# rosielab/emojivoice

Measured on AMD Instinct MI355X. Metric: audio_seconds_per_second, higher is better.
Workload: dtype f32 (deep layers: operand = two block-scaled fp16 pieces, product = 3 fp16 products on the fp16 MFMA, f32 accumulate); 1 GPU; config2: batch 64 x 516-frame (5.99 s) utterances per GPU, 10 Euler steps + HiFi-GAN V1, 22.05 kHz; global_batch=64, frames=516, ode_steps=10, parallelism=dp1, collective=none, batch_pipeline=cfm(i+1) || hifigan(i) on two streams, 2 pipeline(s) in flight

## Files before the change

emojivoice_amd/_lib.py:

```python
from __future__ import annotations

import ctypes as C
import math
import os
import subprocess
from typing import Dict, Optional

import numpy as np
import torch

_HERE = os.path.dirname(os.path.abspath(__file__))
LIB_PATH = os.environ.get("EV_LIB_PATH") or os.path.join(_HERE, "lib", "libemojivoice_hip.so")
CSRC = os.path.join(_HERE, "csrc")
SOURCES = [os.path.join(CSRC, n) for n in ("ev_engine.hip", "ev_kernels.h", "ev_analysis_kernels.h", "ev_analysis.h")] \
    + [os.path.join(os.path.dirname(_HERE), "include", "emojivoice.h")]

EXPORTS = [
    "ev_abi_version", "ev_create", "ev_destroy", "ev_last_error", "ev_load_estimator", "ev_load_vocoder", "ev_load_vocoder_cfg", "ev_load_text_encoder", "ev_text_encoder",
    "ev_text_encoder_status", "ev_stft_magnitude", "ev_denoise", "ev_align", "ev_dbg_conv_bench",
    "ev_workspace_bytes", "ev_cfm_decode", "ev_estimator", "ev_hifigan", "ev_profile_enable", "ev_profile_read", "ev_profile_read_split", "ev_dbg_last_cfg", "ev_set_arithmetic", "ev_get_arithmetic",
    "ev_op_conv1d", "ev_op_groupnorm_mish", "ev_op_groupnorm_mish2", "ev_op_conv_groupnorm", "ev_op_layernorm", "ev_op_split_pieces", "ev_op_attention", "ev_op_ln_mlp", "ev_set_mrf_streams_max",
    "ev_cfm_decode2", "ev_reserve", "ev_alloc_count", "ev_dbg_sk_stats", "ev_op_attn_out", "ev_dbg_set_amax", "ev_dbg_set_attn_h16", "ev_dbg_set_chain", "ev_dbg_sk_taken",
    "ev_load_mel_basis", "ev_mel_spectrogram",
    "ev_maximum_path", "ev_log_prior", "ev_mas_align",
    "ev_estimator_rows", "ev_cfm_loss",
    "ev_load_resampler", "ev_resample", "ev_mel_stats",
    "ev_trim_bounds", "ev_trim_apply",
    "ev_pitch_yin", "ev_dtw",
    "ev_loudness",
    "ev_pyin_observe", "ev_pyin_decode",
    "ev_op_attention2", "ev_op_attn_out2",
    "ev_load_stoi", "ev_stoi",
    "ev_load_stft_dist", "ev_stft_dist",
    "ev_load_voice_quality", "ev_voice_quality",
    "ev_load_formants", "ev_formants", "ev_formant_track",
    "ev_perturbation",
    "ev_load_harmonics", "ev_harmonics",
    "ev_functionals",
    "ev_load_auditory", "ev_auditory",
]


class EvLibraryError(RuntimeError):
    pass

# ... 114 lines not shown
    lib.ev_load_voice_quality.argtypes = [vp, vp, vp, i32, i32, i32, vp, vp, i32, i32, i32, vp, C.c_double]
    lib.ev_voice_quality.argtypes = [vp, vp, vp, i32, i32, C.c_double, vp, vp, vp, vp]
    lib.ev_load_formants.argtypes = [vp, vp, i32, i32, i32, C.c_double, C.c_double, C.c_double, i32]
    lib.ev_formants.argtypes = [vp, vp, vp, i32, i32, C.c_double, vp, vp, vp, vp]
    lib.ev_formant_track.argtypes = [vp, vp, vp, i32, i32, i32, i32, vp, C.c_double, C.c_double, C.c_double, vp, vp, vp, vp, vp]
    lib.ev_perturbation.argtypes = [vp, vp, vp, i32, i32, i32, vp, i32, i32, C.c_double, C.c_double, C.c_double, vp, vp, vp, vp]
    lib.ev_load_harmonics.argtypes = [vp, vp, vp, i32, i32, i32, C.c_double, i32, C.c_double, C.c_double, C.c_double]
    lib.ev_harmonics.argtypes = [vp, vp, vp, i32, i32, vp, vp, vp, i32, C.c_double, vp, vp, vp, vp]
    lib.ev_functionals.argtypes = [vp, vp, vp, vp, i32, i32, i32, vp, i32, vp, vp, vp]
    lib.ev_load_auditory.argtypes = [vp, vp, vp, i32, i32, i32, vp, i32, vp, vp, i32, i32, i32, C.c_double]
    lib.ev_auditory.argtypes = [vp, vp, vp, i32, i32, C.c_double, vp, vp, vp, vp, vp]
    lib.ev_maximum_path.argtypes = [vp, vp, vp, vp, i32, i32, i32, vp, vp, vp]
    lib.ev_log_prior.argtypes = [vp, vp, vp, i32, i32, i32, vp, vp]
    lib.ev_mas_align.argtypes = [vp, vp, vp, vp, vp, i32, i32, i32, vp, vp, vp, vp, vp]
    lib.ev_profile_enable.argtypes = [vp, i32]
    lib.ev_profile_read.argtypes = [vp, C.POINTER(C.c_double), C.POINTER(C.c_double), C.POINTER(C.c_int64), i32]
    lib.ev_profile_read_split.argtypes = [vp, C.POINTER(C.c_double), C.POINTER(C.c_double), C.POINTER(C.c_int64)]
    lib.ev_dbg_last_cfg.argtypes = [vp]
    lib.ev_set_arithmetic.argtypes = [vp, i32]
    lib.ev_get_arithmetic.argtypes = [vp]
    lib.ev_dbg_set_amax.argtypes = [vp, i32]
    lib.ev_dbg_set_attn_h16.argtypes = [vp, i32]
    lib.ev_dbg_set_chain.argtypes = [vp, i32]
    lib.ev_dbg_sk_taken.argtypes = [vp]
    lib.ev_dbg_sk_taken.restype = C.c_int64
    lib.ev_op_conv1d.argtypes = [vp, vp, vp, vp, i32, i32, i32, i32, i32, i32, i32, i32, i32, f32, vp, vp]
    lib.ev_op_groupnorm_mish.argtypes = [vp, vp, vp, vp, vp, i32, i32, i32, i32, vp, vp]
    lib.ev_op_groupnorm_mish2.argtypes = [vp, vp, vp, vp, vp, i32, i32, i32, i32, i32, vp, i32, vp, vp, vp]
    lib.ev_op_conv_groupnorm.argtypes = [vp, vp, vp, vp, i32, i32, i32, vp, vp, vp, i32, vp, vp, vp, vp, vp, C.POINTER(C.c_int), vp]
    lib.ev_op_layernorm.argtypes = [vp, vp, vp, vp, i32, i32, vp, vp]
    lib.ev_op_split_pieces.argtypes = [vp, vp, i32, vp, vp]
    lib.ev_op_attention.argtypes = [vp, vp, vp, i32, i32, i32, vp, vp]
    lib.ev_op_attn_out.argtypes = [vp, vp, vp, i32, i32, vp, vp, vp, vp]
    lib.ev_op_attention2.argtypes = [vp, vp, vp, i32, i32, i32, i32, i32, i32, vp, C.POINTER(C.c_int), vp]
    lib.ev_op_attn_out2.argtypes = [vp, vp, vp, i32, i32, i32, i32, vp, vp, f32, f32, f32, vp, C.POINTER(C.c_int), vp]
    lib.ev_op_ln_mlp.argtypes = [vp, vp, vp, vp, vp, vp, vp, vp, vp, vp, vp, i32, i32, i32, vp, vp]
    for n in EXPORTS:
        getattr(lib, n)
    _lib = lib
    return lib


def _stream_ptr() -> int:
    return int(torch.cuda.current_stream().cuda_stream)


# ... 671 lines not shown
        for b0 in range(0, B, bmax):
            b1 = min(B, b0 + bmax)
            self._check(self.lib.ev_hifigan(self.h, mel[b0:b1].data_ptr(), b1 - b0, T, wav[b0:b1].data_ptr(), _stream_ptr()), "ev_hifigan")
        return wav

    def workspace_bytes(self, B: int, Tp: int, Tv: int) -> int:
        return int(self.lib.ev_workspace_bytes(self.h, B, Tp, Tv))

    def profile_enable(self, on: bool):
        self._check(self.lib.ev_profile_enable(self.h, int(on)), "ev_profile_enable")

    def op_split_pieces(self, x):
        x = self._f32(x).reshape(-1)
        out = torch.empty((3, x.numel()), dtype=torch.float32, device=x.device)
        self._check(self.lib.ev_op_split_pieces(self.h, x.data_ptr(), x.numel(), out.data_ptr(), _stream_ptr()), "ev_op_split_pieces")
        return out

    def set_arithmetic(self, bf16_products: int):
        self._check(self.lib.ev_set_arithmetic(self.h, int(bf16_products)), "ev_set_arithmetic")

    def set_amax(self, on: bool) -> None:
        self._check(self.lib.ev_dbg_set_amax(self.h, int(bool(on))), "ev_dbg_set_amax")

    def set_attn_h16(self, on: bool) -> None:
        self._check(self.lib.ev_dbg_set_attn_h16(self.h, int(bool(on))), "ev_dbg_set_attn_h16")

    def set_chain(self, on: bool) -> None:
        self._check(self.lib.ev_dbg_set_chain(self.h, int(bool(on))), "ev_dbg_set_chain")

    def arithmetic(self) -> int:
        return int(self.lib.ev_get_arithmetic(self.h))

    def last_cfg(self) -> int:
        return int(self.lib.ev_dbg_last_cfg(self.h))

    def profile_read_split(self):
        ms, fl, n = C.c_double(), C.c_double(), C.c_int64()
        self._check(self.lib.ev_profile_read_split(self.h, C.byref(ms), C.byref(fl), C.byref(n)), "ev_profile_read_split")
        return ms.value, fl.value, n.value

    def profile_read(self, reset: bool = True):
        ms, fl, n = C.c_double(), C.c_double(), C.c_int64()
        self._check(self.lib.ev_profile_read(self.h, C.byref(ms), C.byref(fl), C.byref(n), int(reset)), "ev_profile_read")
        return ms.value, fl.value, n.value

    def op_conv1d(self, x, w, bias, dilation=1, transposed=False, stride=1, padding=0, pre_lrelu_slope=-1.0):
# ... 145 lines not shown
```

emojivoice_amd/csrc/ev_engine.hip:

```cpp
#include "ev_kernels.h"
#include "../../include/emojivoice.h"

#include <math.h>
#include <stdlib.h>
#include <stdarg.h>
#include <stdio.h>
#include <string.h>

#include <algorithm>
#include <atomic>
#include <mutex>
#include <numeric>
#include <string>
#include <unordered_map>
#include <vector>

namespace {

struct HostTensor {
    const float* p = nullptr;
    int ndim = 0;
    int64_t shape[4] = {0, 0, 0, 0};
    int64_t numel() const { int64_t n = 1; for (int i = 0; i < ndim; ++i) n *= shape[i]; return n; }
};
// ... 10 lines not shown
    int2* taplist[3] = {nullptr, nullptr, nullptr};
    int* nact[3] = {nullptr, nullptr, nullptr};
    bool sparse_taps = false;
    bool tile128_exact = true;
    int kstack_mt = 0, kstack_tap = 0;
    int ntaps = 0, off[EV_MAX_TAPS] = {0};
    int halo_lo = 0, halo_hi = 0;
    bool wide = false;
    int Cin = 0, Cout = 0, Mpad = 0, Kpad = 0;
    double macs_per_row = 0;
};

struct Epi {
    int act = ACT_NONE; float act_slope = 0.f; const float* act_a = nullptr; const float* act_b = nullptr;
    int mask1 = 0; float scale = 1.f; const float* R = nullptr; int ldr = 0; int accum = 0; int div3 = 0;
    int act2_lrelu = 0; float act2_slope = 0.f; int mask2 = 0; const float* rowmask = nullptr; int mmul = 1;
    float* Y2 = nullptr; int ldy2 = 0;
    float pro_slope = -1.f;
    int dbg = 0; int force_cfg = -1; int stagger = -1; unsigned long long* stamps = nullptr;
    float* gn_part = nullptr;
    int isplit_log2 = 31, isstride = 0;
    unsigned* ymax = nullptr; int ymax_mul = 1; const unsigned* rmax = nullptr; const unsigned* yold = nullptr; const unsigned* xmax = nullptr; int xmax_n = 0;
    int osplit_log2 = 31, osstride = 0;
};

struct ResnetW { ConvLayer c1r, c2; float *g1, *b1, *g2, *b2; };
struct TransW {
    ConvLayer qkv, out, ff1, ff2; float *ln1g, *ln1b, *ln3g, *ln3b, *alpha, *binv;
    float qkv_scale[3] = {0.f, 0.f, 0.f};
};

struct EstimatorW {
    bool loaded = false;
    int in_ch = 0;
    ConvLayer t1, t2, tmlp;
    ResnetW rn[6];
    ConvLayer rn0_c1r_x, rn0_c1r_ms;
    TransW tr[6];
    ConvLayer down0, down1, up0, up1, fin_conv, fin_proj;
    float *fin_g, *fin_b;
};

struct VocoderW {
    bool loaded = false;
    int rb = 1;
    int nl = 4;
// ... 66 lines not shown
    bool use_chain = true;
    bool fuse_mlp = true;
    int gn_stats_tiles = 0;
    int fuse_mlp_min_tiles = 96;
    std::vector<hipEvent_t> ev_pool; size_t ev_used = 0;
    hipStream_t ws_stream = nullptr; bool ws_stream_valid = false;
    float* temb_host[2] = {nullptr, nullptr}; size_t temb_cap[2] = {0, 0}; hipEvent_t temb_ev[2] = {nullptr, nullptr}; int temb_slot = 0;
    float* cap_pool = nullptr; size_t cap_stride = 0; int cap_used = 0; int cap_nt[8] = {0};
    struct TprojEntry { int nt; float* d; };
    std::vector<TprojEntry> tproj_cache;
    bool captured = false; int cap_B = 0, cap_Tp = 0;
    int64_t n_allocs = 0;
    double prof_flops = 0; int64_t prof_launches = 0;
    struct ProfRec { int kind, Cin, Cout, ntaps, nrows, cfg, lean; double flops; bool split = false; };
    std::vector<ProfRec> prof_recs;
    hipStream_t stream = nullptr;
    hipStream_t mrf_stream[2] = {nullptr, nullptr};
    hipEvent_t mrf_ev[4] = {nullptr, nullptr, nullptr, nullptr};
    int ncu = 0;
    unsigned* sk_ctrl = nullptr;
    unsigned sk_seq = 0;
    float* sk_part = nullptr;
    int split_terms = 16;
    bool use_amax = true;
    bool amax_emitted = false;
    int n_fp32_only_layers = 0;
    int last_cfg = -1;
    bool sk_balance = true;
    int sk_wgs = 2;
    int sk_spin = 3000;
    int mrf_max_frames = 16384;
    int force_cfg = -1;
    bool lean = true;
    bool small_sk = true;
    bool sk32_lean = true;
    bool gn_stats = true;
    bool qkv_h16 = true;
    bool attn_sk = true;
    int attn_tpw = 2;
    bool full_rezero = false;
    int rb2_minkeep = 4;
};

namespace {

int fail(ev_handle* h, const char* fmt, ...) {
// ... 352 lines not shown
        launch<conv_gemm_kernel<BM, BN, WM, WN, PF, E == EPI_FULL, (E > 0 ? E : 0)>>(lo.device, dim3(p.mtiles * p.ntiles), dim3(256), smem, st, p);
    });
}

template <int BM, int BN, int WM, int WN, int TERMS = 6>
void launch_split(const ConvParams& p, hipStream_t st, const LaunchOpts& lo) {
    const size_t xs = (size_t)(BN + ((lo.halo + 7) & ~7)) * EVX_RSB;
    constexpr size_t es = (size_t)4 * 32 * (BM / WM + 4) * sizeof(float);
    const size_t smem = xs > es ? xs : es;
    dispatch<1, 2, 3>(epi_flavour(p, true), [&](auto E) {
        launch<conv_split_kernel<BM, BN, WM, WN, E, TERMS>>(lo.device, dim3(p.mtiles * p.ntiles), dim3(256), smem, st, p);
    });
}
template <int BM, int BN, int WM, int WN>
void launch_h16(const ConvParams& p, hipStream_t st, const LaunchOpts& lo) {
    const size_t xs = (size_t)(BN + EV_HALO) * EVH_RSB + 16;
    constexpr size_t es = (size_t)4 * 32 * (BM / WM + 4) * sizeof(float);
    const size_t smem = xs > es ? xs : es;
    const dim3 grid(p.mtiles * p.ntiles);
    if (p.Wq && p.act != ACT_SNAKE)
        dispatch<1, 3>(epi_flavour(p, true), [&](auto E) { launch<conv_h16_kernel<BM, BN, WM, WN, E, 1>>(lo.device, grid, dim3(256), smem, st, p); });
    else dispatch<1, 2, 3>(epi_flavour(p, true), [&](auto E) { launch<conv_h16_kernel<BM, BN, WM, WN, E>>(lo.device, grid, dim3(256), smem, st, p); });
}
inline bool split_ok(const ConvLayer& L, const ConvParams& p0) {
    ConvParams p = p0;
    p.dbg &= ~4;
    return L.Wx && lean_ok(p) && (p.isplit_log2 >= 31 || (p.isplit_log2 >= 6 && p.isplit_log2 < 31)) && L.Cin % EVX_KC == 0 && L.Cin == L.Kpad && L.Mpad % 128 == 0 && ((size_t)p.bias & 15) == 0;
}

template <int TW>
void launch_sk(const ConvParams& p, hipStream_t st, const LaunchOpts& lo) {
    constexpr int KS = TW == 4 ? 4 : 8, BN = TW == 4 ? 64 : 32;
    const int nchunks = p.Kpad / EV_BK, rows = BN + ((lo.halo + 7) & ~7);
    int kbs = nchunks < (TW == 4 ? 8 : 32) ? nchunks : (TW == 4 ? 8 : 32);
    while (kbs > 8 && ((size_t)rows * (32 * kbs + 4) * 4 > 150 * 1024 || rows * kbs * 8 > EV_SK_MAXF4(TW))) kbs = (kbs - 1) & ~7;
    const size_t xs = 2 * EV_MAX_TAPS + (size_t)rows * (32 * kbs + 4);
    const size_t red = (size_t)(KS - 1) * TW * 16 * 64, es = (size_t)TW * 32 * 36;
    size_t smem = std::max(xs, std::max(red, es)) * sizeof(float);
    ConvParams q = p;
    q.sk_kb = kbs;
    dispatch<1, 2, 3, 0, EPI_FULL>(epi_flavour(p, lo.lean && lean_ok(p)), [&](auto E) {
        launch<conv_gemm_sk_kernel<KS, E == EPI_FULL, (E > 0 ? E : 0), TW>>(lo.device, dim3(p.mtiles * p.ntiles), dim3(64 * TW * KS), smem, st, q);
    });
}

constexpr int EV_CAPTURE_SLOTS = 8;
// ... 35 lines not shown
    else if constexpr (PIPE == PIPE_BF16)
        dispatch<1, 3>(lean, [&](auto E) { launch<conv_split_bal_kernel<BM, BN, WM, WN, E>>(lo.device, grid, block, smem, h->stream, p); });
    else if (BN + p.halo_lo + p.halo_hi <= 16 * 9)
        dispatch<1, 3>(lean, [&](auto E) { launch<conv_h16_bal_kernel<BM, BN, WM, WN, E, 9>>(lo.device, grid, block, smem, h->stream, p); });
    else dispatch<1, 3>(lean, [&](auto E) { launch<conv_h16_bal_kernel<BM, BN, WM, WN, E>>(lo.device, grid, block, smem, h->stream, p); });
    return 0;
}
inline bool split_bal_ok(const ev_handle* h, const ConvLayer& L, const ConvParams& p, long nwg, int wpc) {
    return h->sk_balance && h->ncu > 0 && split_ok(L, p) && p.act != ACT_SNAKE && !p.dbg && !p.stamps && !p.gn_part &&
           nwg * 2 >= h->ncu && wpc * h->ncu <= EV_SK_MAXWG && (long)nwg * (p.Kpad / EVX_KC) >= (long)wpc * h->ncu;
}
inline bool bal_ok(const ev_handle* h, const ConvLayer& L, const ConvParams& p, long nwg, int wpc) {
    if (L.sparse_taps) return false;
    return h->sk_balance && h->ncu > 0 && lean_ok(p) && p.act != ACT_SNAKE && !p.dbg && !p.stamps && !p.gn_part &&
           nwg >= h->ncu && nwg < 4L * wpc * h->ncu && wpc * h->ncu <= EV_SK_MAXWG && (long)nwg * (p.Kpad / EV_BK) >= (long)wpc * h->ncu;
}

enum : int {
    CFG_128x128 = 0, CFG_64x128 = 1, CFG_32x256 = 2, CFG_64x192 = 5, CFG_64x64 = 6,
    CFG_64x64_PF = 8,
    CFG_SK64 = 9, CFG_SK32 = 19,
    CFG_SPLIT = 40, CFG_SPLIT64 = 41, CFG_SPLIT3 = 43, CFG_SPLIT9 = 49,
    CFG_H16 = 46,
    CFG_SPLIT_BAL = 60,
    CFG_H16_64 = 47, CFG_BAL64 = 56, CFG_H16_BAL = 66,
};
struct ConvTile { int cfg, bm, bn, slots; bool split; };
constexpr ConvTile EV_TILES[] = {
    {CFG_128x128, 128, 128, 3, false}, {CFG_64x128, 64, 128, 4, false}, {CFG_32x256, 32, 256, 3, false}, {CFG_64x192, 64, 192, 4, false},
    {CFG_64x64, 64, 64, 5, false}, {CFG_64x64_PF, 64, 64, 5, false}, {CFG_SK64, 64, 64, 0, false}, {CFG_SK32, 32, 32, 0, false},
    {CFG_SPLIT, 128, 128, 0, true}, {CFG_SPLIT64, 64, 128, 0, true}, {CFG_SPLIT3, 128, 128, 0, true}, {CFG_H16, 128, 128, 0, true},
    {CFG_SPLIT9, 128, 128, 0, true}, {CFG_SPLIT_BAL, 128, 128, 0, true},
};
inline const ConvTile* conv_tile(int cfg) {
    for (const ConvTile& t : EV_TILES) if (t.cfg == cfg) return &t;
    return nullptr;
}
inline int tile_list(const ConvTile& t) { return t.bm == 128 ? 0 : t.bm == 64 ? 1 : 2; }
inline int tile_mtiles(const ConvTile& t, const ConvLayer& L) { return t.bm == 128 ? L.Mpad / 128 : (L.Cout + t.bm - 1) / t.bm; }
inline long tile_count(const ConvTile& t, const ConvLayer& L, const Geom& g) { return (long)tile_mtiles(t, L) * ((g.nrows + t.bn - 1) / t.bn); }

int pick_cfg(const ev_handle* h, const ConvLayer& L, const ConvParams& p, const Geom& g) {
    auto tiles = [&](int cfg) { return tile_count(*conv_tile(cfg), L, g); };
    int cfg;
    if (L.Cout <= 32) cfg = CFG_32x256;
    else {
        double best = 1e30;
        cfg = CFG_64x128;
        for (int c : {CFG_64x128, CFG_64x192, CFG_64x64}) {
            const ConvTile& k = *conv_tile(c);
            const long nwg = tiles(c);
            const double w = (double)(k.bm / 32) * (k.bn / 32);
            double t;
            if (nwg <= 256L * k.slots) t = (double)((nwg + 255) / 256) * w;
            else t = (double)nwg * w / 256.0 + (nwg < 256L * k.slots * 3 ? w : 0.0);
            t *= (c == CFG_64x64 ? 1.08 : 1.0);
            if (t < best - 1e-9) { best = t; cfg = c; }
        }
    }
    if (L.sparse_taps && L.Cout > 32 && tiles(CFG_64x64) <= 256L * 5 * 2) cfg = CFG_64x64;
    if (cfg == CFG_64x64 && tiles(CFG_64x64) <= 320) cfg = CFG_64x64_PF;
    if (cfg == CFG_64x128 && L.Cout % 128 == 0 && !L.sparse_taps && tiles(CFG_64x128) >= 256L * 4 * 6)
        cfg = (L.Cin > 128 && L.ntaps >= 7) ? CFG_64x192 : CFG_128x128;
// ... 35 lines not shown
            p.plane_bytes = (L.Mpad / 32) * (L.Kpad / 8) * 1024; p.koff0 = L.off[0]; p.kdoff = d;
            if (!L.sparse_taps) p.ktaps_n = L.ntaps;
            else { p.kstack_mt = L.kstack_mt; p.kstack_tap = L.kstack_tap; }
        }
    }
    p.halo_lo = L.halo_lo; p.halo_hi = L.halo_hi;
    p.pro_lrelu = e.pro_slope >= 0.f; p.pro_slope = e.pro_slope;
    p.act = e.act; p.act_slope = e.act_slope; p.act_a = e.act_a; p.act_b = e.act_b;
    p.mask1 = e.mask1; p.scale = e.scale; p.R = e.R; p.ldr = e.ldr; p.accum = e.accum; p.div3 = e.div3;
    p.act2_lrelu = e.act2_lrelu; p.act2_slope = e.act2_slope; p.mask2 = e.mask2; p.rowmask = e.rowmask;
    p.Y2 = e.Y2; p.ldy2 = e.ldy2; p.dbg = e.dbg; p.stamps = e.stamps;
    p.xmax = e.xmax; p.xmax_n = e.xmax_n; p.rmax = e.rmax; p.yold = e.yold; p.ymax_mul = e.ymax_mul; h->amax_emitted = false;
    if ((ldx & 3) || (L.Cin & 3)) return fail(h, "conv input must be float4-aligned (ldx %d Cin %d)", ldx, L.Cin);
    if (over_4gib(g, ldx) || over_4gib(g, ldy) || (e.R && over_4gib(g, e.ldr)) || (e.Y2 && over_4gib(g, e.ldy2)))
        return fail(h, "tensor of %.1f GiB exceeds the 4 GiB buffer-addressing limit: split the batch", (double)g.nrows * std::max(ldx, ldy) * 4.0 / 1073741824.0);

    int cfg = pick_cfg(h, L, p, g);
    LaunchOpts lo;
    lo.device = h->device; lo.lean = h->lean; lo.halo = L.halo_lo + L.halo_hi;
    if (h->force_cfg >= 0) cfg = h->force_cfg;
    if (e.force_cfg >= 0) { cfg = e.force_cfg < 1000 ? e.force_cfg % 100 : -1; lo.wgs_per_cu = (e.force_cfg / 100) % 10; }
    if ((h->force_cfg >= 0 || e.force_cfg >= 0) && !conv_tile(cfg))
        return fail(h, "launch_conv: forced tile configuration %d is not one launch_conv selects", e.force_cfg >= 0 ? e.force_cfg : h->force_cfg);
    if (prof_begin(h)) return 1;
    {
        const ConvTile& s = *conv_tile(cfg == CFG_SK64 ? CFG_32x256 : cfg);
        p.stagger_slots = tile_count(s, L, g) >= 256L * s.slots * 3 ? s.slots : 0;
        if (e.stagger >= 0) p.stagger_slots = e.stagger;
    }
    if (conv_tile(cfg)->split && !split_ok(L, p)) cfg = CFG_128x128;
    if (cfg == CFG_H16 && !L.Wh) cfg = CFG_SPLIT;
    const bool fp16 = h->split_terms == 16 && L.Wh;
    {
        const bool lean1or3 = lean_ok(p) && p.act != ACT_SNAKE && h->lean;
        const bool h16 = cfg == CFG_H16 || (cfg == CFG_SPLIT64 && fp16);
        const bool gemm = (cfg == CFG_128x128 || cfg == CFG_64x128 || cfg == CFG_64x192 || cfg == CFG_64x64) && lean1or3;
        const bool no_amax = !h->use_amax;
        if (!no_amax && e.ymax && lean1or3 && (h16 || gemm) && (!e.R || e.rmax) && (!e.accum || e.yold)) { p.ymax = e.ymax; h->amax_emitted = true; }
        if (no_amax) p.xmax = nullptr;
    }
    const ConvTile& t = *conv_tile(cfg);
    p.mtiles = tile_mtiles(t, L); p.ntiles = (g.nrows + t.bn - 1) / t.bn;
    p.taplist = L.taplist[tile_list(t)]; p.nact_tab = L.nact[tile_list(t)]; p.tl_stride = L.sparse_taps ? EV_MAX_TAPS : 0;
    switch (cfg) {
    case CFG_H16: launch_h16<128, 128, 2, 2>(p, h->stream, lo); break;
    case CFG_SPLIT64:
        if (fp16) { launch_h16<64, 128, 2, 2>(p, h->stream, lo); cfg = CFG_H16_64; }
        else if (h->split_terms == 3) launch_split<64, 128, 2, 2, 3>(p, h->stream, lo);
        else launch_split<64, 128, 2, 2, 6>(p, h->stream, lo);
        break;
    case CFG_SPLIT_BAL:
        if (fp16) { if (launch_bal<PIPE_H16, 128, 128, 2, 2>(h, p, lo, 2)) return 1; cfg = CFG_H16_BAL; }
        else if (launch_bal<PIPE_BF16, 128, 128, 2, 2>(h, p, lo, 2)) return 1;
        break;
    case CFG_SPLIT: launch_split<128, 128, 2, 2, 6>(p, h->stream, lo); break;
    case CFG_SPLIT3: launch_split<128, 128, 2, 2, 3>(p, h->stream, lo); break;
    case CFG_SPLIT9: launch_split<128, 128, 2, 2, 9>(p, h->stream, lo); break;
    case CFG_128x128: launch_cfg<128, 128, 2, 2>(p, h->stream, lo); break;
    case CFG_64x128: launch_cfg<64, 128, 2, 2>(p, h->stream, lo); break;
    case CFG_64x192: launch_cfg<64, 192, 2, 2>(p, h->stream, lo); break;
    case CFG_64x64_PF: launch_cfg<64, 64, 2, 2, true>(p, h->stream, lo); break;
    case CFG_SK64: launch_sk<4>(p, h->stream, lo); break;
    case CFG_SK32: {
        const int xr = 32 + p.halo_lo + p.halo_hi;
        const bool fast = h->sk32_lean && h->lean && lean_ok(p) && (p.ktaps_n > 0 || p.kstack_mt > 0) && p.isplit_log2 >= 31 && !p.pro_lrelu && p.Cin == p.Kpad &&
                          (p.Kpad == 128 || p.Kpad == 256 || p.Kpad == 512 || p.Kpad == 1024) && (ldx % 4) == 0 && xr <= 16 * (512 / (p.Kpad / 4)) && (size_t)g.nrows * ldx * 4 < ((size_t)1 << 31) &&
                          (size_t)xr * (p.Kpad + 4) * 4 <= 150 * 1024;
        if (!fast) { launch_sk<1>(p, h->stream, lo); break; }
// ... 939 lines not shown
}

extern "C" {

int ev_abi_version(void) { return EV_ABI_VERSION; }

int ev_create(ev_handle** out, int device, const ev_model_dims* dims) {
    if (!out || !dims) return 1;
    *out = nullptr;
    int ndev = 0;
    if (hipGetDeviceCount(&ndev) != hipSuccess || device < 0 || device >= ndev) return 2;
    if (hipSetDevice(device) != hipSuccess) return 3;
    ev_handle* h = new ev_handle();
    h->device = device;
    h->dims = *dims;
    { const char* fp = getenv("EV_FUSE_PAIRS"); if (fp && *fp == '0') h->fuse_pairs = false; }
    { const char* fp = getenv("EV_FUSE_MLP"); if (fp && *fp == '0') h->fuse_mlp = false; }
    { const char* fp = getenv("EV_FUSE_ATTN"); if (fp && *fp == '0') h->fuse_attn = false; }
    if (getenv("EV_NO_ATTN_H16")) h->attn_h16 = false;
    if (getenv("EV_NO_CHAIN")) h->use_chain = false;
    { const char* fp = getenv("EV_FUSE_MLP_MIN"); if (fp && *fp) h->fuse_mlp_min_tiles = atoi(fp); }
    { const char* fp = getenv("EV_MRF_STREAMS_MAX"); if (fp && *fp) h->mrf_max_frames = atoi(fp); }
    if (getenv("EV_NO_AMAX")) h->use_amax = false;
    { const char* sp = getenv("EV_SPLIT"); if (sp && *sp) { const int t = atoi(sp); h->split_terms = (t == 0 || t == 3 || t == 6 || t == 9 || t == 16) ? t : 16; } }
    { const char* fp = getenv("EV_NO_SK_BALANCE"); if (fp && *fp && *fp != '0') h->sk_balance = false; }
    { const char* fp = getenv("EV_SK_SPIN"); if (fp && *fp) h->sk_spin = atoi(fp); }
    { const char* fp = getenv("EV_SK_WGS"); if (fp && *fp) h->sk_wgs = std::min(3, std::max(1, atoi(fp))); }
    { const char* fp = getenv("EV_FORCE_CFG"); if (fp && *fp) h->force_cfg = atoi(fp); }
    if (getenv("EV_NO_LEAN")) h->lean = false;
    if (getenv("EV_NO_SK")) h->small_sk = false;
    if (getenv("EV_NO_SK32_LEAN")) h->sk32_lean = false;
    if (getenv("EV_NO_GN_STATS")) h->gn_stats = false;
    if (getenv("EV_NO_QKV_H16")) h->qkv_h16 = false;
    if (getenv("EV_NO_ATTN_SK")) h->attn_sk = false;
    { const char* fp = getenv("EV_ATTN_TPW"); if (fp) h->attn_tpw = std::max(1, atoi(fp)); }
    if (getenv("EV_FULL_REZERO")) h->full_rezero = true;
    { const char* fp = getenv("EV_RB2_MINKEEP"); if (fp) h->rb2_minkeep = atoi(fp); }
    if (hipDeviceGetAttribute(&h->ncu, hipDeviceAttributeMultiprocessorCount, device) != hipSuccess) h->ncu = 0;
    if (dims->n_feats != 80 || dims->channels != 256 || dims->head_dim != 64 || dims->heads != 2) {
        delete h;
        return 4;
    }
    *out = h;
    return 0;
}

// ... 765 lines not shown
    int cin = w.ch[0];
    const bool ms = mrf_streams_for(h, B, T) && !h->prof && v.Pax[0][1] != nullptr;
    if (ms && !h->mrf_stream[0]) {
        for (int c = 0; c < 2; ++c) HIPCHK(h, hipStreamCreateWithFlags(&h->mrf_stream[c], hipStreamNonBlocking));
        for (int c = 0; c < 4; ++c) HIPCHK(h, hipEventCreateWithFlags(&h->mrf_ev[c], hipEventDisableTiming));
    }
    if (ms) HIPCHK(h, hipStreamSynchronize(h->stream));
    hipStream_t s0 = h->stream;
    struct StreamGuard {
        ev_handle* h; hipStream_t s; bool bal; bool ms; bool done;
        ~StreamGuard() {
            h->stream = s; h->sk_balance = bal;
            if (ms && !done) { for (int c = 0; c < 2; ++c) if (h->mrf_stream[c]) (void)hipStreamSynchronize(h->mrf_stream[c]); }
        }
    } guard{h, s0, h->sk_balance, ms, false};
    if (ms) h->sk_balance = false;
    const int nl = w.nl;
    for (int i = 0; i < nl; ++i) {
        const int l = i + 1, C = w.ch[l], s = w.ups[i].Cout / C;
        const float next_slope = (l == nl) ? 0.01f : 0.1f;
        {
            Epi e;
            with_slots(e, xin, nullptr, v.U[l], s);
            if (launch_conv(h, w.ups[i], xin, cin, v.U[l], s * C, v.g[l - 1], e)) return 1;
            wrote(v.U[l], false);
        }
        if (ms) {
            HIPCHK(h, hipEventRecord(h->mrf_ev[3], s0));
            for (int c = 0; c < 2; ++c) HIPCHK(h, hipStreamWaitEvent(h->mrf_stream[c], h->mrf_ev[3], 0));
        }
        for (int j = 0; j < 3; ++j) {
            const float* x = v.U[l];
            const bool own = ms && j > 0;
            h->stream = own ? h->mrf_stream[j - 1] : s0;
            float* pp[2] = {own ? v.Pax[j - 1][l] : v.Pa[l], own ? v.Pbx[j - 1][l] : v.Pb[l]};
            float* t1 = own ? v.T1x[j - 1][l] : v.T1[l];
            if (w.rb == 2) {
                const int b = i * 3 + j;
                auto join = [&](Epi& e) {
                    e.accum = (j > 0);
                    if (j == 2) { e.div3 = 1; e.act2_lrelu = 1; e.act2_slope = next_slope; }
                };
                if (rb2_ok(h, w.c1[b], C)) {
                    if (ms && j > 0) HIPCHK(h, hipStreamWaitEvent(h->stream, h->mrf_ev[j - 1], 0));
                    Epi e; join(e);
                    float* y = v.XS[l];
// ... 31 lines not shown
                e2.accum = (j > 0);
                if (j == 2) { e2.div3 = 1; e2.act2_lrelu = 1; e2.act2_slope = next_slope; }
                if (l < nl) with_slots(e2, x, nullptr, y, 1);
                if (launch_chain(h, w.c1[i * 3 + j], w.c2[i * 3 + j], x, y, C, v.g[l], e2)) return 1;
                wrote(y, e2.accum != 0);
                if (ms) HIPCHK(h, hipEventRecord(h->mrf_ev[j], h->stream));
                continue;
            }
            for (int mm = 0; mm < 3; ++mm) {
                if (ms && mm == 2 && j > 0) HIPCHK(h, hipStreamWaitEvent(h->stream, h->mrf_ev[j - 1], 0));
                Epi e2; e2.R = x; e2.ldr = C;
                float* y = pp[mm & 1];
                if (mm == 2) {
                    y = v.XS[l];
                    e2.accum = (j > 0);
                    if (j == 2) { e2.div3 = 1; e2.act2_lrelu = 1; e2.act2_slope = next_slope; }
                }
                if (h->fuse_pairs && (C == 32 || C == 64 || (C == 128 && w.c1[i * 3 + j][mm].ntaps <= 3))) {
                    if (mm == 2 && l < nl) with_slots(e2, x, nullptr, y, 1);
                    if (launch_pair(h, w.c1[i * 3 + j][mm], w.c2[i * 3 + j][mm], x, y, C, v.g[l], e2)) return 1;
                    wrote(y, e2.accum != 0);
                } else {
                    Epi e1; e1.pro_slope = 0.1f; e1.act = ACT_LRELU; e1.act_slope = 0.1f;
                    with_slots(e1, x, nullptr, t1, 1);
                    if (launch_conv(h, w.c1[i * 3 + j][mm], x, C, t1, C, v.g[l], e1)) return 1;
                    wrote(t1, false);
                    with_slots(e2, t1, x, y, 1);
                    if (launch_conv(h, w.c2[i * 3 + j][mm], t1, C, y, C, v.g[l], e2)) return 1;
                    wrote(y, e2.accum != 0);
                }
                if (ms && mm == 2) HIPCHK(h, hipEventRecord(h->mrf_ev[j], h->stream));
                x = y;
            }
        }
        h->stream = s0;
        if (ms) HIPCHK(h, hipStreamWaitEvent(s0, h->mrf_ev[2], 0));
        xin = v.XS[l];
        cin = C;
    }
    {
        const Geom& g4 = v.g[nl];
        const int Cl = w.ch[nl];
        if ((Cl == 32 || Cl == 16 || Cl == 8) && w.post_k == 7 && w.post_w && g4.P >= 3) {
            const int tiles = (g4.T + 255) / 256;
            const dim3 grid((unsigned)(B * tiles));
            if (Cl == 32) hipLaunchKernelGGL((conv_post_kernel<32, 7>), grid, dim3(256), 0, h->stream, (const float*)v.XS[nl], (const float*)w.post_w, w.post_b, d_wav, g4.T, g4.S, g4.P);
// ... 49 lines not shown
                            a.n, a.ms, a.fl / (a.ms * 1e9));
                fclose(f);
            }
        }
    }
    if (conv_ms) *conv_ms = ms;
    if (conv_flops) *conv_flops = h->prof_flops;
    if (conv_launches) *conv_launches = h->prof_launches;
    if (reset) { h->ev_used = 0; h->prof_flops = 0; h->prof_launches = 0; h->prof_recs.clear(); }
    return 0;
}

int ev_dbg_last_cfg(ev_handle* h) { return h ? h->last_cfg : -1; }

int ev_set_arithmetic(ev_handle* h, int bf16_products) {
    if (!h) return 1;
    if (bf16_products != 0 && bf16_products != 3 && bf16_products != 6 && bf16_products != 9 && bf16_products != 16)
        return fail(h, "ev_set_arithmetic: 0, 3, 6, 9 or 16, got %d", bf16_products);
    h->split_terms = bf16_products;
    return 0;
}
int ev_get_arithmetic(ev_handle* h) { return h ? h->split_terms : -1; }

int ev_dbg_set_amax(ev_handle* h, int on) {
    if (!h) return 1;
    h->use_amax = on != 0;
    return 0;
}

int ev_dbg_set_chain(ev_handle* h, int on) {
    if (!h) return 1;
    h->use_chain = on != 0;
    return 0;
}

int ev_dbg_set_attn_h16(ev_handle* h, int on) {
    if (!h) return 1;
    h->attn_h16 = on != 0;
    return 0;
}

int ev_profile_read_split(ev_handle* h, double* ms_out, double* flops_out, int64_t* launches_out) {
    if (!h) return 1;
    HIPCHK(h, hipStreamSynchronize(h->stream));
    double ms = 0, fl = 0;
    int64_t n = 0;
// ... 406 lines not shown
```

emojivoice_amd/csrc/ev_kernels.h:

```cpp
#pragma once
#include <hip/hip_runtime.h>
#include <stdint.h>
#include <type_traits>

typedef float f32x16 __attribute__((ext_vector_type(16)));
typedef float f32x4 __attribute__((ext_vector_type(4)));
typedef int i32x4 __attribute__((ext_vector_type(4)));

#define EV_MAX_TAPS 16
#define EV_BK 32
#define EV_LDK 36
#define EV_WROWS 128
#define EV_SK_MAXF4(TW) ((TW) == 4 ? (64 + 64) * 8 * 8 : 16 * 512)
#define EV_HALO 64

enum { ACT_NONE = 0, ACT_LRELU = 1, ACT_TANH = 2, ACT_SILU = 3, ACT_MISH = 4, ACT_SNAKE = 5 };

struct SkCtl {
    unsigned* ctrl;
    unsigned* flags;
    float* part;
    int part_floats;
    int q, r;
    int spin_limit;
// ... 1417 lines not shown
                const bool have_next = !(last_tap && ch + 1 == nchunks);
                const unsigned nap = have_next ? q_off(ntv.x, last_tap ? ch * 2 + 2 : ch * 2) : q_off(tv_first.x, 0);
                ldQB(QB1, brow, 1);
                __builtin_amdgcn_sched_barrier(0);
                mmaQ(QA0, QB0);
                __builtin_amdgcn_sched_barrier(0);
                ldQA(QA0, nap);
                ldQB(QB0, nbrow, 0);
                __builtin_amdgcn_sched_barrier(0);
                mmaQ(QA1, QB1);
                __builtin_amdgcn_sched_barrier(0);
                ldQA(QA1, nap + 2048u);
                brow = nbrow;
            }
        }
#pragma unroll
        for (int a = 0; a < QM; ++a)
#pragma unroll
            for (int b = 0; b < QN; ++b) acc[a][b] *= acc_out;
        __builtin_amdgcn_s_setprio(3);
        ev_amax_from_acc_q<QM, QN>(p, am, acc, c.row0(n0), lane);
        conv_epilogue_lean_q<TM, TN, LEAN>(p, acc, c.epi(smem), c.ch0(m0), c.row0(n0), lane);
        ev_amax_emit(p, am, c.row0(n0), TN * 32, lane);
    }
}

template <int BM, int BN, int WAVES_M, int WAVES_N, int LEAN, int TERMS = 6>
__global__ __launch_bounds__(256, 2) void conv_split_bal_kernel(const ConvParams p) {
    constexpr int TM = BM / WAVES_M / 32;
    constexpr int TN = BN / WAVES_N / 32;
    static_assert(WAVES_M * WAVES_N == 4 && TM >= 1 && TN >= 1 && LEAN != 0, "balanced build: 4 waves, lean epilogue");
    extern __shared__ __attribute__((aligned(16))) float smem[];
    char* Xb = (char*)smem;
    const int tid = threadIdx.x;
    const int lane = tid & 63;
    const int wave = __builtin_amdgcn_readfirstlane(tid >> 6);
    const int wm = wave / WAVES_N, wn = wave % WAVES_N;
    const int li = lane & 31, lh = lane >> 5;
    const int nchunks = p.Kpad / EVX_KC;
    const int g = blockIdx.x;
    const unsigned tag = sk_tag(p.sk);
    int u = sk_start(p.sk, g);
    const int ue = sk_start(p.sk, g + 1);
    const __amdgpu_buffer_rsrc_t rPart = ev_rsrc(p.sk.part), rW = ev_rsrc(p.Wx), rX = ev_rsrc(p.X);
    const unsigned pslot = (unsigned)p.sk.part_floats * 8u;
    constexpr int PN = TM * TN * 4;
// ... 4142 lines not shown
```

include/emojivoice.h:

```cpp
#ifndef EMOJIVOICE_H
#define EMOJIVOICE_H

#include <stddef.h>
#include <stdint.h>

#ifdef __cplusplus
extern "C" {
#endif

#define EV_ABI_VERSION 4

typedef struct ev_handle ev_handle;

typedef struct ev_tensor_index {
    const char *name;
    uint64_t offset;
    int32_t ndim;
    int64_t shape[4];
} ev_tensor_index;

typedef struct ev_model_dims {
    int32_t n_feats;
    int32_t spk_emb_dim;
    int32_t channels;
// ... 149 lines not shown
int ev_functionals(ev_handle *h, const double *d_v , const uint8_t *d_mask ,
                   const int32_t *d_len , int B, int K, int F,
                   const double *q , int NQ,
                   double *d_stat , int32_t *d_count , void *stream);

int ev_load_auditory(ev_handle *h, const double *window , const double *twiddle , int W, int H, int nfft,
                     const double *mel_w , int n_mel, const double *eq ,
                     const double *dct , int n_ceps, int k_lo, int k_hi, double compress );
int ev_auditory(ev_handle *h, const float *d_x , const int32_t *d_len , int B, int L, double power_floor,
                double *d_frame , double *d_mfcc , int32_t *d_flags ,
                double *d_bands , void *stream);

int ev_profile_enable(ev_handle *h, int on);
int ev_profile_read(ev_handle *h, double *conv_ms, double *conv_flops, int64_t *conv_launches, int reset);
int ev_profile_read_split(ev_handle *h, double *ms, double *flops, int64_t *launches);
int ev_set_arithmetic(ev_handle *h, int setting);
int ev_get_arithmetic(ev_handle *h);

int ev_dbg_last_cfg(ev_handle *h);

int ev_dbg_conv_bench(ev_handle *h, int Cin, int Cout, int K, int dil, int B, int T, int P, int iters, int dbg, int cfg, float *ms_out);

int ev_dbg_set_amax(ev_handle *h, int on);
int ev_dbg_set_attn_h16(ev_handle *h, int on);
int ev_dbg_set_chain(ev_handle *h, int on);

int ev_dbg_sk_stats(ev_handle *h, uint32_t *out3);
int64_t ev_dbg_sk_taken(ev_handle *h);

int ev_op_conv1d(ev_handle *h, const float *d_x , const float *w ,
                 const float *bias , int B, int Cin, int T, int Cout, int K, int dilation,
                 int transposed, int stride, int padding, float pre_lrelu_slope , float *d_y, void *stream);
int ev_op_groupnorm_mish(ev_handle *h, const float *d_x , const float *d_gamma, const float *d_beta,
                         const int32_t *d_lengths, int B, int C, int T, int groups, float *d_y, void *stream);
int ev_op_groupnorm_mish2(ev_handle *h, const float *d_x , const float *d_gamma, const float *d_beta,
                          const int32_t *d_lengths, int B, int C, int T, int groups, int mode, const float *d_temb,
                          int temb_stride, const float *d_R, float *d_y, void *stream);
int ev_op_conv_groupnorm(ev_handle *h, const float *d_x , const float *w ,
                         const float *bias , int Cin, int T, int K, const float *d_gamma,
                         const float *d_beta, const int32_t *d_lengths , int mode, const float *d_temb, const float *d_R,
                         float *d_conv, float *d_part, float *d_y, int *tiles_out, void *stream);
int ev_op_split_pieces(ev_handle *h, const float *d_x, int n, float *d_pieces, void *stream);
int ev_op_layernorm(ev_handle *h, const float *d_x , const float *d_gamma, const float *d_beta, int rows,
                    int C, float *d_y, void *stream);
int ev_op_ln_mlp(ev_handle *h, const float *d_x, const float *d_ln_g, const float *d_ln_b, const float *w1, const float *b1,
                 const float *d_alpha_exp, const float *d_beta_inv, const float *w2, const float *b2, const float *d_rowmask,
// ... 17 lines not shown
```

Baseline: 4837 audio_s/s.

## Add LDS-resident fp16 conv kernel for HiFi-GAN upsample and MRF layers

Adds conv_h16_res_kernel, which stages the whole input row tile (all Cin channels plus halo), split into fp16 pieces, into LDS once. It then loops over every output-channel pass and tap from LDS, instead of re-streaming input chunks for each K chunk and M tile. The kernel is selected by default for HiFi-GAN upsample and resblock conv1 layers with Cin 128 or 256 and a small enough halo when the H16 config would have been chosen. This is meant to cut global memory reloads and pipeline overhead. In exchange it uses large LDS allocations, which may lower occupancy, and it adds a debug toggle and an env var to turn it off.

```diff
diff --git a/emojivoice_amd/_lib.py b/emojivoice_amd/_lib.py
--- a/emojivoice_amd/_lib.py
+++ b/emojivoice_amd/_lib.py
@@ -20,7 +20,7 @@
     "ev_text_encoder_status", "ev_stft_magnitude", "ev_denoise", "ev_align", "ev_dbg_conv_bench",
     "ev_workspace_bytes", "ev_cfm_decode", "ev_estimator", "ev_hifigan", "ev_profile_enable", "ev_profile_read", "ev_profile_read_split", "ev_dbg_last_cfg", "ev_set_arithmetic", "ev_get_arithmetic",
     "ev_op_conv1d", "ev_op_groupnorm_mish", "ev_op_groupnorm_mish2", "ev_op_conv_groupnorm", "ev_op_layernorm", "ev_op_split_pieces", "ev_op_attention", "ev_op_ln_mlp", "ev_set_mrf_streams_max",
-    "ev_cfm_decode2", "ev_reserve", "ev_alloc_count", "ev_dbg_sk_stats", "ev_op_attn_out", "ev_dbg_set_amax", "ev_dbg_set_attn_h16", "ev_dbg_set_chain", "ev_dbg_sk_taken",
+    "ev_cfm_decode2", "ev_reserve", "ev_alloc_count", "ev_dbg_sk_stats", "ev_op_attn_out", "ev_dbg_set_amax", "ev_dbg_set_attn_h16", "ev_dbg_set_chain", "ev_dbg_sk_taken", "ev_dbg_set_conv_resident",
     "ev_load_mel_basis", "ev_mel_spectrogram",
     "ev_maximum_path", "ev_log_prior", "ev_mas_align",
     "ev_estimator_rows", "ev_cfm_loss",
@@ -181,6 +181,7 @@
     lib.ev_dbg_set_amax.argtypes = [vp, i32]
     lib.ev_dbg_set_attn_h16.argtypes = [vp, i32]
     lib.ev_dbg_set_chain.argtypes = [vp, i32]
+    lib.ev_dbg_set_conv_resident.argtypes = [vp, i32]
     lib.ev_dbg_sk_taken.argtypes = [vp]
     lib.ev_dbg_sk_taken.restype = C.c_int64
     lib.ev_op_conv1d.argtypes = [vp, vp, vp, vp, i32, i32, i32, i32, i32, i32, i32, i32, i32, f32, vp, vp]
@@ -898,6 +899,9 @@
     def set_amax(self, on: bool) -> None:
         self._check(self.lib.ev_dbg_set_amax(self.h, int(bool(on))), "ev_dbg_set_amax")
 
+    def set_conv_resident(self, on: bool) -> None:
+        self._check(self.lib.ev_dbg_set_conv_resident(self.h, int(bool(on))), "ev_dbg_set_conv_resident")
+
     def set_attn_h16(self, on: bool) -> None:
         self._check(self.lib.ev_dbg_set_attn_h16(self.h, int(bool(on))), "ev_dbg_set_attn_h16")
 
diff --git a/emojivoice_amd/csrc/ev_engine.hip b/emojivoice_amd/csrc/ev_engine.hip
--- a/emojivoice_amd/csrc/ev_engine.hip
+++ b/emojivoice_amd/csrc/ev_engine.hip
@@ -56,6 +56,7 @@
     int isplit_log2 = 31, isstride = 0;
     unsigned* ymax = nullptr; int ymax_mul = 1; const unsigned* rmax = nullptr; const unsigned* yold = nullptr; const unsigned* xmax = nullptr; int xmax_n = 0;
     int osplit_log2 = 31, osstride = 0;
+    bool resident = false;
 };
 
 struct ResnetW { ConvLayer c1r, c2; float *g1, *b1, *g2, *b2; };
@@ -168,6 +169,7 @@
     unsigned sk_seq = 0;
     float* sk_part = nullptr;
     int split_terms = 16;
+    bool conv_resident = true;
     bool use_amax = true;
     bool amax_emitted = false;
     int n_fp32_only_layers = 0;
@@ -566,6 +568,14 @@
         dispatch<1, 3>(epi_flavour(p, true), [&](auto E) { launch<conv_h16_kernel<BM, BN, WM, WN, E, 1>>(lo.device, grid, dim3(256), smem, st, p); });
     else dispatch<1, 2, 3>(epi_flavour(p, true), [&](auto E) { launch<conv_h16_kernel<BM, BN, WM, WN, E>>(lo.device, grid, dim3(256), smem, st, p); });
 }
+template <int CIN, int BM, int BN, int WM, int WN>
+void launch_h16_res(ConvParams p, hipStream_t st, const LaunchOpts& lo) {
+    const size_t xs = (size_t)(BN + lo.halo) * (4 * CIN + 16) + 16;
+    constexpr size_t es = (size_t)4 * 32 * (BM / WM + 4) * sizeof(float);
+    const size_t smem = p.Mpad / BM > 1 ? xs + es : (xs > es ? xs : es);
+    p.ntiles = (p.nrows + BN - 1) / BN;
+    dispatch<1, 3>(epi_flavour(p, true), [&](auto E) { launch<conv_h16_res_kernel<CIN, BM, BN, WM, WN, E>>(lo.device, dim3(p.ntiles), dim3(256), smem, st, p); });
+}
 inline bool split_ok(const ConvLayer& L, const ConvParams& p0) {
     ConvParams p = p0;
     p.dbg &= ~4;
@@ -647,6 +657,7 @@
     CFG_SK64 = 9, CFG_SK32 = 19,
     CFG_SPLIT = 40, CFG_SPLIT64 = 41, CFG_SPLIT3 = 43, CFG_SPLIT9 = 49,
     CFG_H16 = 46,
+    CFG_H16_RES = 48,
     CFG_SPLIT_BAL = 60,
     CFG_H16_64 = 47, CFG_BAL64 = 56, CFG_H16_BAL = 66,
 };
@@ -655,7 +666,7 @@
     {CFG_128x128, 128, 128, 3, false}, {CFG_64x128, 64, 128, 4, false}, {CFG_32x256, 32, 256, 3, false}, {CFG_64x192, 64, 192, 4, false},
     {CFG_64x64, 64, 64, 5, false}, {CFG_64x64_PF, 64, 64, 5, false}, {CFG_SK64, 64, 64, 0, false}, {CFG_SK32, 32, 32, 0, false},
     {CFG_SPLIT, 128, 128, 0, true}, {CFG_SPLIT64, 64, 128, 0, true}, {CFG_SPLIT3, 128, 128, 0, true}, {CFG_H16, 128, 128, 0, true},
-    {CFG_SPLIT9, 128, 128, 0, true}, {CFG_SPLIT_BAL, 128, 128, 0, true},
+    {CFG_SPLIT9, 128, 128, 0, true}, {CFG_SPLIT_BAL, 128, 128, 0, true}, {CFG_H16_RES, 128, 128, 0, true},
 };
 inline const ConvTile* conv_tile(int cfg) {
     for (const ConvTile& t : EV_TILES) if (t.cfg == cfg) return &t;
@@ -664,6 +675,14 @@
 inline int tile_list(const ConvTile& t) { return t.bm == 128 ? 0 : t.bm == 64 ? 1 : 2; }
 inline int tile_mtiles(const ConvTile& t, const ConvLayer& L) { return t.bm == 128 ? L.Mpad / 128 : (L.Cout + t.bm - 1) / t.bm; }
 inline long tile_count(const ConvTile& t, const ConvLayer& L, const Geom& g) { return (long)tile_mtiles(t, L) * ((g.nrows + t.bn - 1) / t.bn); }
+
+inline bool conv_resident_ok(const ConvLayer& L, const ConvParams& p) {
+    if (!L.Wq || !L.Wh || p.act == ACT_SNAKE || !split_ok(L, p) || (L.sparse_taps && !(L.tile128_exact && L.kstack_mt == 0))) return false;
+    const int halo = L.halo_lo + L.halo_hi;
+    if (L.Cin == 128) return L.Mpad == 128 && L.Cout == 128 && halo <= 27;
+    if (L.Cin == 256) return L.Mpad % 256 == 0 && L.Cout == L.Mpad && halo <= 14;
+    return false;
+}
 
 int pick_cfg(const ev_handle* h, const ConvLayer& L, const ConvParams& p, const Geom& g) {
     auto tiles = [&](int cfg) { return tile_count(*conv_tile(cfg), L, g); };
@@ -745,6 +764,10 @@
     if (e.force_cfg >= 0) { cfg = e.force_cfg < 1000 ? e.force_cfg % 100 : -1; lo.wgs_per_cu = (e.force_cfg / 100) % 10; }
     if ((h->force_cfg >= 0 || e.force_cfg >= 0) && !conv_tile(cfg))
         return fail(h, "launch_conv: forced tile configuration %d is not one launch_conv selects", e.force_cfg >= 0 ? e.force_cfg : h->force_cfg);
+    if (cfg == CFG_H16 && e.resident && h->conv_resident && conv_resident_ok(L, p) && L.Mpad <= 256) cfg = CFG_H16_RES;
+    else if (cfg == CFG_H16_RES && !conv_resident_ok(L, p))
+        return fail(h, "launch_conv: forced tile configuration 48 (conv_h16_res_kernel) does not fit this layer: Cin %d Cout %d halo %d (Cin = Cout = 128 with halo <= 27, or Cin = 256 with halo <= 14)",
+                    L.Cin, L.Cout, L.halo_lo + L.halo_hi);
     if (prof_begin(h)) return 1;
     {
         const ConvTile& s = *conv_tile(cfg == CFG_SK64 ? CFG_32x256 : cfg);
@@ -756,7 +779,7 @@
     const bool fp16 = h->split_terms == 16 && L.Wh;
     {
         const bool lean1or3 = lean_ok(p) && p.act != ACT_SNAKE && h->lean;
-        const bool h16 = cfg == CFG_H16 || (cfg == CFG_SPLIT64 && fp16);
+        const bool h16 = cfg == CFG_H16 || cfg == CFG_H16_RES || (cfg == CFG_SPLIT64 && fp16);
         const bool gemm = (cfg == CFG_128x128 || cfg == CFG_64x128 || cfg == CFG_64x192 || cfg == CFG_64x64) && lean1or3;
         const bool no_amax = !h->use_amax;
         if (!no_amax && e.ymax && lean1or3 && (h16 || gemm) && (!e.R || e.rmax) && (!e.accum || e.yold)) { p.ymax = e.ymax; h->amax_emitted = true; }
@@ -767,6 +790,10 @@
     p.taplist = L.taplist[tile_list(t)]; p.nact_tab = L.nact[tile_list(t)]; p.tl_stride = L.sparse_taps ? EV_MAX_TAPS : 0;
     switch (cfg) {
     case CFG_H16: launch_h16<128, 128, 2, 2>(p, h->stream, lo); break;
+    case CFG_H16_RES:
+        if (L.Cin == 128) launch_h16_res<128, 128, 128, 2, 2>(p, h->stream, lo);
+        else launch_h16_res<256, 256, 64, 4, 1>(p, h->stream, lo);
+        break;
     case CFG_SPLIT64:
         if (fp16) { launch_h16<64, 128, 2, 2>(p, h->stream, lo); cfg = CFG_H16_64; }
         else if (h->split_terms == 3) launch_split<64, 128, 2, 2, 3>(p, h->stream, lo);
@@ -1752,6 +1779,7 @@
     { const char* fp = getenv("EV_FUSE_MLP_MIN"); if (fp && *fp) h->fuse_mlp_min_tiles = atoi(fp); }
     { const char* fp = getenv("EV_MRF_STREAMS_MAX"); if (fp && *fp) h->mrf_max_frames = atoi(fp); }
     if (getenv("EV_NO_AMAX")) h->use_amax = false;
+    { const char* fp = getenv("EV_NO_CONV_RESIDENT"); if (fp && *fp && *fp != '0') h->conv_resident = false; }
     { const char* sp = getenv("EV_SPLIT"); if (sp && *sp) { const int t = atoi(sp); h->split_terms = (t == 0 || t == 3 || t == 6 || t == 9 || t == 16) ? t : 16; } }
     { const char* fp = getenv("EV_NO_SK_BALANCE"); if (fp && *fp && *fp != '0') h->sk_balance = false; }
     { const char* fp = getenv("EV_SK_SPIN"); if (fp && *fp) h->sk_spin = atoi(fp); }
@@ -2563,6 +2591,7 @@
         {
             Epi e;
             with_slots(e, xin, nullptr, v.U[l], s);
+            e.resident = true;
             if (launch_conv(h, w.ups[i], xin, cin, v.U[l], s * C, v.g[l - 1], e)) return 1;
             wrote(v.U[l], false);
         }
@@ -2640,6 +2669,7 @@
                     wrote(y, e2.accum != 0);
                 } else {
                     Epi e1; e1.pro_slope = 0.1f; e1.act = ACT_LRELU; e1.act_slope = 0.1f;
+                    e1.resident = e2.resident = true;
                     with_slots(e1, x, nullptr, t1, 1);
                     if (launch_conv(h, w.c1[i * 3 + j][mm], x, C, t1, C, v.g[l], e1)) return 1;
                     wrote(t1, false);
@@ -2735,6 +2765,11 @@
 }
 int ev_get_arithmetic(ev_handle* h) { return h ? h->split_terms : -1; }
 
+int ev_dbg_set_conv_resident(ev_handle* h, int on) {
+    if (!h) return 1;
+    h->conv_resident = on != 0;
+    return 0;
+}
 int ev_dbg_set_amax(ev_handle* h, int on) {
     if (!h) return 1;
     h->use_amax = on != 0;
diff --git a/emojivoice_amd/csrc/ev_kernels.h b/emojivoice_amd/csrc/ev_kernels.h
--- a/emojivoice_amd/csrc/ev_kernels.h
+++ b/emojivoice_amd/csrc/ev_kernels.h
@@ -1463,6 +1463,173 @@
         ev_amax_from_acc_q<QM, QN>(p, am, acc, c.row0(n0), lane);
         conv_epilogue_lean_q<TM, TN, LEAN>(p, acc, c.epi(smem), c.ch0(m0), c.row0(n0), lane);
         ev_amax_emit(p, am, c.row0(n0), TN * 32, lane);
+    }
+}
+
+template <int CIN, int BM, int BN, int WAVES_M, int WAVES_N, int LEAN>
+__global__ __launch_bounds__(256, 2) void conv_h16_res_kernel(const ConvParams p) {
+    using Core = EvConvCore<BM, BN, WAVES_M, WAVES_N, EvPipeH16>;
+    constexpr int TM = Core::TM, TN = Core::TN, RPS = Core::RPS;
+    static_assert(TM == 2 && TN == 2 && CIN % (2 * EVX_KC) == 0 && 128 % BN == 0, "64 x 64 wave tiles, chunk pairs, tiles inside a 128-row tile");
+    constexpr int RSB = 4 * CIN + 16, NCH = CIN / EVX_KC, KG32 = CIN / 32;
+    constexpr int HMAX = (80 * 1024) / RSB - BN;
+    constexpr int XPASS = (BN + HMAX + RPS - 1) / RPS;
+    constexpr int QM = 2 * TM, QN = 2 * TN;
+    extern __shared__ __attribute__((aligned(16))) float smem[];
+    char* Xb = (char*)smem;
+
+    const int n0 = ev_xcd_remap(blockIdx.x, p.ntiles) * BN;
+    const int n128 = n0 & ~127;
+    if (ev_tile_is_padding(p.S, p.P, p.T, p.nrows, n128, 128)) return;
+    Core c(p, 0);
+    const int lane = c.lane, wave = c.wave, srow = c.srow, sc4 = c.sc4;
+    const int xrows = BN + p.halo_lo + p.halo_hi;
+    const int mpass = p.Mpad / BM;
+    float* red = (float*)(Xb + xrows * RSB);
+    float* Es = (mpass > 1 ? red + 4 : smem) + wave * (32 * (TM * 32 + 4));
+    EvAmax am = ev_amax_begin(p, c.row0(n0), TN * 32);
+    const __amdgpu_buffer_rsrc_t rX = ev_rsrc(p.X), rQ = ev_rsrc(p.Wq);
+    const unsigned wlane = c.wlane;
+    const int f16i = lane & 15, kg = lane >> 4;
+    auto ldQA = [&](f32x4 (&dst)[2][QM], unsigned aoff) {
+#pragma unroll
+        for (int pc = 0; pc < 2; ++pc)
+#pragma unroll
+            for (int a = 0; a < QM; ++a) dst[pc][a] = ev_bload4(rQ, wlane, aoff + (unsigned)(a * KG32 * 2048 + pc * 1024));
+    };
+    f32x4 QA0[2][QM], QA1[2][QM], QB0[2][QN], QB1[2][QN];
+    int chw = c.ch0(0);
+    int nact;
+    int2 tlv, tv_first;
+    unsigned qbase;
+    auto q_off = [&](int tap_bytes, int kg32) -> unsigned { return (unsigned)tap_bytes + qbase + (unsigned)kg32 * 2048u; };
+    auto pass_begin = [&](int mp) {
+        chw = c.ch0(mp * BM);
+        const int mt = chw >> 7;
+        nact = __builtin_amdgcn_readfirstlane(p.nact_tab ? p.nact_tab[mt] : p.ntaps);
+        const int2* tl = p.taplist + (size_t)mt * p.tl_stride;
+        tlv = (lane < nact) ? tl[lane] : make_int2(0, 0);
+        tv_first = ev_tap_at(tlv, 0);
+        qbase = (unsigned)((chw >> 4) * KG32) * 2048u;
+        const unsigned a0 = q_off(tv_first.x, 0);
+        ldQA(QA0, a0); ldQA(QA1, a0 + 2048u);
+    };
+    pass_begin(0);
+
+    float xs;
+    {
+        const int lo = n128 - p.halo_lo, rows128 = 128 + p.halo_lo + p.halo_hi, scan_rows = (rows128 + RPS - 1) & ~(RPS - 1);
+        auto scan = [&](auto finite_only) -> float {
+            constexpr bool FIN = decltype(finite_only)::value;
+            float mx = 0.f;
+            for (int r = srow; r < scan_rows; r += RPS) {
+                const unsigned ro = ev_row_off(p, lo + r, true, sc4);
+                for (int ch = 0; ch < NCH; ++ch) {
+                    const f32x4 v = ev_bload4(rX, ro, ev_chunk_off<EVX_KC>(p, ch));
+                    mx = fmaxf(mx, FIN ? evh_absmax4_finite(v) : evh_absmax4(v));
+                }
+            }
+            return evh_wg_max(red, 0, wave, lane, mx);
+        };
+        float mx = p.xmax ? ev_amax_read(p, lo, lo + rows128 - 1, lane) : -1.f;
+        if (mx < 0.f) mx = scan(std::false_type{});
+        if (!evh_is_finite(mx)) {
+            if (!p.xmax) ev_lds_barrier();
+            mx = scan(std::true_type{});
+        }
+        xs = evh_scale_for(mx);
+    }
+    const float acc_in = p.wh_scale * xs;
+    const float acc_out = 1.0f / acc_in;
+
+    {
+        unsigned xoff[XPASS];
+        ev_row_offs<RPS>(p, n0 - p.halo_lo + srow, xrows, sc4, xoff);
+        __builtin_amdgcn_s_setprio(3);
+#pragma unroll 1
+        for (int ch = 0; ch < NCH; ch += 2) {
+            const unsigned soff0 = ev_chunk_off<EVX_KC>(p, ch), soff1 = ev_chunk_off<EVX_KC>(p, ch + 1);
+            f32x4 xg[2][XPASS];
+#pragma unroll
+            for (int q = 0; q < XPASS; ++q) { xg[0][q] = ev_bload4(rX, xoff[q], soff0); xg[1][q] = ev_bload4(rX, xoff[q], soff1); }
+#pragma unroll
+            for (int k = 0; k < 2; ++k)
+#pragma unroll
+                for (int q = 0; q < XPASS; ++q) {
+                    const int r = q * RPS + srow;
+                    uint2 q0v, q1v;
+                    evh_split4(ev_pro_lrelu4(p, xg[k][q]) * xs, q0v, q1v);
+                    if (r < xrows) {
+                        char* dst = Xb + r * RSB + (ch + k) * (4 * EVX_KC) + sc4 * 2;
+                        *(uint2*)(dst) = q0v; *(uint2*)(dst + EVX_KC * 2) = q1v;
+                    }
+                }
+        }
+        ev_lds_barrier();
+        __builtin_amdgcn_s_setprio(0);
+    }
+
+    auto ldQB = [&](f32x4 (&dst)[2][QN], const char* brow, int ks) {
+#pragma unroll
+        for (int pc = 0; pc < 2; ++pc)
+#pragma unroll
+            for (int b = 0; b < QN; ++b) dst[pc][b] = *(const f32x4*)(brow + b * 16 * RSB + pc * (EVX_KC * 2) + ks * 64);
+    };
+    const char* qbb = Xb + (c.wn * (TN * 32) + f16i + p.halo_lo) * RSB + 16 * kg;
+    for (int mp = 0; mp < mpass; ++mp) {
+        if (mp > 0) pass_begin(mp);
+        f32x4 acc[QM][QN];
+#pragma unroll
+        for (int a = 0; a < QM; ++a) {
+            f32x4 bq = {0.f, 0.f, 0.f, 0.f};
+            const int c0 = chw + a * 16 + 4 * kg;
+            if (p.bias && c0 < p.Cout) bq = *(const f32x4*)(p.bias + c0) * acc_in;
+#pragma unroll
+            for (int b = 0; b < QN; ++b) acc[a][b] = bq;
+        }
+        auto mmaQ = [&](const f32x4 (&a)[2][QM], const f32x4 (&b)[2][QN]) {
+            constexpr int PA[3] = {0, 1, 0}, PB[3] = {1, 0, 0};
+#pragma unroll
+            for (int t = 0; t < 3; ++t)
+#pragma unroll
+                for (int i = 0; i < QM; ++i)
+#pragma unroll
+                    for (int jj = 0; jj < QN; ++jj)
+                        acc[i][jj] = __builtin_amdgcn_mfma_f32_16x16x32_f16(__builtin_bit_cast(f16x8, a[PA[t]][i]), __builtin_bit_cast(f16x8, b[PB[t]][jj]), acc[i][jj], 0, 0, 0);
+        };
+        const char* first = qbb + tv_first.y * RSB;
+        const char* brow = first;
+        ldQB(QB0, brow, 0);
+#pragma unroll 1
+        for (int ch = 0; ch < NCH; ++ch) {
+            for (int ti = 0; ti < nact; ++ti) {
+                const bool last_tap = (ti + 1 == nact);
+                const int2 ntv = last_tap ? tv_first : ev_tap_at(tlv, ti + 1);
+                const bool have_next = !(last_tap && ch + 1 == NCH);
+                const char* nbrow = have_next ? qbb + ntv.y * RSB + (last_tap ? ch + 1 : ch) * (4 * EVX_KC) : first;
+                const unsigned nap = have_next ? q_off(ntv.x, last_tap ? ch * 2 + 2 : ch * 2) : q_off(tv_first.x, 0);
+                ldQB(QB1, brow, 1);
+                __builtin_amdgcn_sched_barrier(0);
+                mmaQ(QA0, QB0);
+                __builtin_amdgcn_sched_barrier(0);
+                ldQA(QA0, nap);
+                ldQB(QB0, nbrow, 0);
+                __builtin_amdgcn_sched_barrier(0);
+                mmaQ(QA1, QB1);
+                __builtin_amdgcn_sched_barrier(0);
+                ldQA(QA1, nap + 2048u);
+                brow = nbrow;
+            }
+        }
+#pragma unroll
+        for (int a = 0; a < QM; ++a)
+#pragma unroll
+            for (int b = 0; b < QN; ++b) acc[a][b] *= acc_out;
+        __builtin_amdgcn_s_setprio(3);
+        ev_amax_from_acc_q<QM, QN>(p, am, acc, c.row0(n0), lane);
+        conv_epilogue_lean_q<TM, TN, LEAN>(p, acc, Es, chw, c.row0(n0), lane);
+        ev_amax_emit(p, am, c.row0(n0), TN * 32, lane);
+        __builtin_amdgcn_s_setprio(0);
     }
 }
 
diff --git a/include/emojivoice.h b/include/emojivoice.h
--- a/include/emojivoice.h
+++ b/include/emojivoice.h
@@ -195,6 +195,7 @@
 int ev_dbg_conv_bench(ev_handle *h, int Cin, int Cout, int K, int dil, int B, int T, int P, int iters, int dbg, int cfg, float *ms_out);
 
 int ev_dbg_set_amax(ev_handle *h, int on);
+int ev_dbg_set_conv_resident(ev_handle *h, int on);
 int ev_dbg_set_attn_h16(ev_handle *h, int on);
 int ev_dbg_set_chain(ev_handle *h, int on);
 
```

Result: no change. 4862 audio_s/s (median of 6 runs) (+0.5%).
